# vasudeva-ram/Julia-NewtonRaphsonHANK

Hardware: AMD Instinct MI355X
Metric: sequence-space JVPs/sec (household block: BackwardIteration+ForwardIteration+aggregation, Krusell-Smith T=300) (higher is better)
Workload: dtype f64; 1 GPU; ks_2000x11_T300_N32; grid=2000x11, T=300, tangents_per_gpu=32, step=1 dual-sweep pass: primal + N tangents (hank_primal_jvp), parallelism=tangent-sharded x1

## Files before the change

include/hank_hip.h:

```cpp
#ifndef HANK_HIP_H
#define HANK_HIP_H

#include <stdint.h>

#ifdef __cplusplus
extern "C" {
#endif

typedef struct hank_ctx hank_ctx;

enum {
    HANK_OK = 0,
    HANK_ERR_NO_DEVICE = 1,
    HANK_ERR_BAD_ARG = 2,
    HANK_ERR_KNOTS = 3,
    HANK_ERR_DOMAIN = 4,
    HANK_ERR_NOT_READY = 5,
    HANK_ERR_NONMONOTONE = 6,
    HANK_ERR_NOMEM = 7,
    HANK_ERR_SWEEP = 8,
    HANK_ERR_LAUNCH = 9
};

enum {
// ... 28 lines not shown
int hank_primal(hank_ctx *ctx, const double *xhh, double *agg_out);
int hank_jvp(hank_ctx *ctx, const double *dxhh, int32_t N, double *dagg_out);

int hank_primal_dev(hank_ctx *ctx, const double *d_xhh, double *d_agg_out);
int hank_jvp_dev(hank_ctx *ctx, const double *d_dxhh, int32_t N, double *d_dagg_out);
int hank_check(hank_ctx *ctx);

int hank_primal_jvp(hank_ctx *ctx, const double *xhh, const double *dxhh, int32_t N, double *agg_out,
                    double *dagg_out);
int hank_primal_jvp_dev(hank_ctx *ctx, const double *d_xhh, const double *d_dxhh, int32_t N,
                        double *d_agg_out, double *d_dagg_out);

int hank_get_policy_seq(hank_ctx *ctx, double *out);
int hank_get_dpolicy_seq(hank_ctx *ctx, int32_t N, double *out);
int hank_get_lottery_record(hank_ctx *ctx, int32_t *lo, double *lw, double *ig, void *lq, double *iga);
int hank_get_het_outputs(hank_ctx *ctx, int32_t n_het, const double *dxhh, int32_t N, double *agg_out, double *dagg_out);
int hank_get_het_outputs_dev(hank_ctx *ctx, int32_t n_het, const double *d_dxhh, int32_t N, double *d_agg_out, double *d_dagg_out);
int hank_set_het_outputs(hank_ctx *ctx, int32_t n_het);
int hank_get_grid_aggregates(hank_ctx *ctx, double *agg2_out, int32_t N, double *dagg2_out);
int hank_get_grid_aggregates_dev(hank_ctx *ctx, double *d_agg2_out, int32_t N, double *d_dagg2_out);
int hank_get_dist_seq(hank_ctx *ctx, double *out);

int hank_backward_step(hank_ctx *ctx, const double *value_next, const double *xhh_t,
                       double *value_out, double *policy_out);
int hank_backward_step_dual(hank_ctx *ctx, const double *value_next, const double *dvalue_next,
                            const double *xhh_t, const double *dxhh_t, int32_t N,
                            double *value_out, double *dvalue_out, double *policy_out,
                            double *dpolicy_out);
int hank_forward_step(hank_ctx *ctx, const double *policy, const double *D_prev, double *D_out,
                      double *agg_out);
// ... 64 lines not shown
```

julia-newtonraphsonhank_amd/csrc/hank_device.h:

```cpp
#pragma once
#include <hip/hip_runtime.h>
#include <stdint.h>
#include "hank_geom.h"

#ifndef HANK_XFWD_LQ
#define HANK_XFWD_LQ 1
#endif
#ifndef HANK_XFWD_EARLY_BATCH
#define HANK_XFWD_EARLY_BATCH 0
#endif

namespace hank {

struct Consts {
    int n_a, n_e, G, P;
    int n_hh;
    int diet;
    double beta, gamma, bc;
    const double *a, *z, *Pi;
};

struct Record {
    double *s, *kc, *A, *B, *u, *v, *pol, *lw, *ig, *Dseq;
    int *ib, *lo, *start, *clo;
// ... 487 lines not shown
template <typename VT>
struct AdjHx<VT, 0> {};

struct SsCtl { int stop, iters; double resid; };

enum { ERR_KNOTS = 3, ERR_DOMAIN = 4, ERR_NONMONO = 6 };

__device__ inline void set_err(int *err, int code, int t, int e, int j) {
    if (atomicCAS(&err[0], 0, code) == 0) {
        err[1] = t;
        err[2] = e;
        err[3] = j;
    }
}

__device__ __forceinline__ void lottery_body(const Consts &c, const Record &R, int col, int *err, int write_seg, int use_ib, int *shlo, int *sh_clo, int4 *lq = nullptr) {
    const int t = col / c.n_e, e = col % c.n_e;
    const size_t base = (size_t)col * c.n_a;
    const int n = c.n_a;
    if (threadIdx.x == 0) *sh_clo = 0;
    __syncthreads();
    for (int j = threadIdx.x; j < n; j += blockDim.x) {
        const double p = R.pol[base + j];
        int lo = -1, hi = n;
        if (use_ib) {
            const int g0 = min(max(R.ib[base + j], 0), n - 2);
            const double a0 = c.a[g0], a1 = c.a[g0 + 1];
            if (a0 < p && p <= a1) { lo = g0; hi = g0 + 1; }
            else if (g0 > 0 && p <= a0 && c.a[g0 - 1] < p) { lo = g0 - 1; hi = g0; }
        }
// ... 2 lines not shown
            if (c.a[mid] < p) lo = mid; else hi = mid;
        }
        int l;
        double w, ig;
        if (hi == 0) {
            l = 0; w = 0.0; ig = 0.0;
            atomicMax(sh_clo, j + 1);
        } else if (hi >= n) {
            l = n - 2; w = 1.0; ig = 0.0;
        } else {
            l = hi - 1;
            const double gap = c.a[hi] - c.a[l];
            w = (p - c.a[l]) / gap;
            ig = 1.0 / gap;
        }
        R.lo[base + j] = l; R.lw[base + j] = w; R.ig[base + j] = ig;
        if (lq) lq[base + j] = make_int4(__double2loint(w), __double2hiint(w), l, (hi == 0 || hi >= n) ? 1 : 0);
        shlo[j] = (hi == 0) ? -1 : l;
    }
    __syncthreads();
    const int clo = *sh_clo;
    if (threadIdx.x == 0) R.clo[col] = clo;
    int *st = R.start + (size_t)col * (n + 1);
    int *shst = shlo + n;
    for (int j = threadIdx.x; j < n; j += blockDim.x) {
        const int prev = j ? shlo[j - 1] : -1, cur = shlo[j];
        if (cur < prev) set_err(err, ERR_NONMONO, t, e, j);
        for (int r = (prev < 0 ? 0 : prev + 1); r <= cur; r++) shst[r] = j;
        if (j == n - 1)
            for (int r = (cur < 0 ? 0 : cur + 1); r <= n; r++) shst[r] = n;
    }
    __syncthreads();
    for (int r = threadIdx.x; r <= n; r += blockDim.x) st[r] = shst[r];
    if (write_seg)
        for (int r = threadIdx.x; r < n; r += blockDim.x)
            R.seg[base + r] = make_int4(r > 0 ? shst[r - 1] : shst[r], shst[r], shst[r + 1], 0);
}

struct AdjLane { int e, nl, rl, RB, m; bool mok; };
__device__ __forceinline__ AdjLane adj_lane(const AdjGeom &g) {
    AdjLane L;
    const int lane = threadIdx.x & 63;
    L.e = __builtin_amdgcn_readfirstlane((int)(threadIdx.x >> 6));
    L.nl = lane & (g.NC - 1); L.rl = lane >> g.lgNC; L.RB = 64 >> g.lgNC;
    L.m = blockIdx.y * g.NC + L.nl;
    L.mok = L.m < g.MV;
    return L;
}

template <typename VT, typename Load, typename Begin, typename Src>
__device__ __forceinline__ void adj_dist_body(const Consts &c, const Record &R, const AdjGeom &g, const AdjLane &L, int t, double *adj_sh, Load load,
// ... 152 lines not shown
```

julia-newtonraphsonhank_amd/csrc/hank_hip.hip:

```cpp
#include "hank_kernels.h"
#include "hank_xsweep.h"
#include "hank_xspec.h"
#include "hank_jacobian.h"
#include "hank_wide.h"
#include "hank_hetx.h"
#include "hank_scen.h"
#include "hank_ssbatch.h"
#include "hank_adjoint.h"
#include "hank_boundary.h"
#include "hank_ssdiff_launch.h"
#include "../../include/hank_hip.h"

#include <cstdarg>
#include <cstdio>
#include <cstdlib>
#include <cstring>
#include <initializer_list>
#include <list>
#include <mutex>
#include <new>
#include <vector>

using namespace hank;

// ... 69 lines not shown
    DevBuf<double> dagg_pass;
    DevBuf<double> dagg_cm;
};
struct XWork {
    bool ready = false;
    int grid = 0, Sact = 0, maxt = 768, dmax = XD_MAX;
    DevBuf<XSync> sync;
    DevBuf<double> st_s, st_ds, st_D, st_dD;
    DevBuf<double> Dvirt, aggpart, rho;
    DevBuf<double> D0own;
    DevBuf<int> srcB, srcF;
    DevBuf<int2> unitsF;
    DevBuf<int> unit_overflow;
    int ucap = 64;
    bool rng_valid = false;
    bool neigh = true;
    bool syncwave = true;
    int lds_max = 65536;
    int fault_where = 7;
    int fault = 0;
    bool src_valid = false;
    std::list<XTan> tans;
    int last_blocks = 0;
    int xspec = XSPEC_CRRA;
    int inst[4] = {-1, -1, -1, -1};
};

struct WTan {
    int N = 0;
    DevBuf<double> dxhh;
// ... 94 lines not shown
    int schedule = 2;
    bool forced_xcd = false;
    TanBatch batch;
    int xjvp_max = 64;
    XWork xw;
    struct { DevBuf<double> dpT, iota, E, Cp, F, Dv, W, dsum; int N = 0, n_het = 0; } fn;
    int wide_mode = 0, wide_min = 80, num_cus = 256, wide_r = 2;
    size_t lds_max = 65536;
    DevBuf<char> rec_slab;
    size_t rec_bytes = 0;
    int4 *rec_lq = nullptr;
    double *rec_iga = nullptr;
    DevBuf<int> d_ibw;
    bool seg_valid = true;
    bool lwg_valid = true;
    long long lwg_builds = 0;
    bool wprep_valid = false;
    std::list<WTan> wtans;
    std::list<CotWork> cws;
    CotBatch cot;
    DevBuf<int> d_adj_sb;
    bool adj_seg_valid = false;
    DevBuf<double> d_bnd_q;
    HxRecord hx;
    ScenWork scen;
    int scen_pending = 0;
    std::vector<double> h_Pi, h_z;
    long long stats[N_STATS] = {};
    bool memo_on = true;
    bool xdual_back = true;
// ... 15 lines not shown
static void cot_none(hank_ctx *ctx) { ctx->cot = CotBatch(); }
static void cot_ran(hank_ctx *ctx, const void *ws, int M, const double *pbar) { ctx->cot = CotBatch{true, M, ws, pbar}; }
static void batch_ran(hank_ctx *ctx, int family, const void *ws, int N, const double *dagg_cm, const double *dpol, const std::vector<XPass> *passes = nullptr) {
    ctx->batch = TanBatch{family, true, N, ws, dagg_cm, dpol, passes};
}
static void batch_ran_boundary(hank_ctx *ctx, const void *ws, int N, const double *dagg_cm, const double *dpol, const double *zm) {
    batch_ran(ctx, 0, ws, N, dagg_cm, dpol);
    ctx->batch.boundary = true;
    ctx->batch.bnd_zm = zm;
}
static int batch_current(hank_ctx *ctx, int N, const TanBatch **out) {
    if (!ctx->batch.current || ctx->batch.N != N) return fail(ctx, HANK_ERR_NOT_READY, "no tangent sweep with N=%d is current", N);
    *out = &ctx->batch;
    return HANK_OK;
}
static void record_rewritten(hank_ctx *ctx, bool seg_written, bool lwg_written) {
    ctx->primal_done = true; ctx->seg_valid = seg_written; ctx->lwg_valid = lwg_written;
    ctx->wprep_valid = false; ctx->xw.src_valid = false; ctx->xw.rng_valid = false; ctx->adj_seg_valid = false; ctx->hx.valid = false;
    batch_none(ctx);
    cot_none(ctx);
}
static void record_gone(hank_ctx *ctx) {
    record_rewritten(ctx, false, false);
    ctx->primal_done = false;
}
static hipError_t join_side(hank_ctx *ctx) {
    if (!ctx->side_pending) return hipSuccess;
    ctx->side_pending = false;
    return hipStreamWaitEvent(ctx->stream, ctx->ev_side, 0);
}

static int fail(hank_ctx *ctx, int code, const char *fmt, ...) {
// ... 446 lines not shown
    HIPC(ctx, hipMemsetAsync(X.sync, 0, sizeof(XSync) * ((size_t)2 + 2 * XPASS_MAX), ctx->stream));
    HIPC(ctx, X.st_s.alloc(2 * XG * G));
    HIPC(ctx, X.st_ds.alloc(2 * XG * G * X.dmax));
    const size_t GM = (size_t)c.n_e * X.Sact * 64;
    HIPC(ctx, X.st_D.alloc(2 * XG * std::max(GV, GM)));
    HIPC(ctx, X.st_dD.alloc(2 * XG * GM * xslots(X.dmax + 1).SP));
    HIPC(ctx, X.Dvirt.alloc(P * c.n_e * 64));
    HIPC(ctx, X.D0own.alloc(P * c.n_e));
    HIPC(ctx, X.aggpart.alloc(2 * P * (size_t)X.Sact));
    HIPC(ctx, X.rho.alloc(P));
    HIPC(ctx, X.srcB.alloc(P * X.Sact));
    HIPC(ctx, X.srcF.alloc(P * X.Sact));
    HIPC(ctx, X.unitsF.alloc(P * X.Sact * XUCAP));
    HIPC(ctx, X.unit_overflow.alloc(1));
    HIPC(ctx, hipMemsetAsync(X.unit_overflow, 0, sizeof(int), ctx->stream));
    if (const char *ng = getenv("HANK_XNEIGH")) X.neigh = atoi(ng) != 0;
    if (const char *uc = getenv("HANK_XUCAP")) X.ucap = std::min(XUCAP, std::max(1, atoi(uc)));
    {
        double ms = 20.0;
        if (const char *wm = getenv("HANK_XWAIT_MS")) ms = atof(wm);
        const unsigned long long ticks = (unsigned long long)(std::max(ms, 0.01) * 1e5);
        HIPC(ctx, hipMemcpyToSymbol(HIP_SYMBOL(hank::g_xwait_ticks), &ticks, sizeof(ticks)));
    }
    if (const char *sv = getenv("HANK_XSYNCWAVE")) X.syncwave = atoi(sv) != 0;
    X.lds_max = (int)prop.sharedMemPerBlock;
    if (const char *xf = getenv("HANK_XFAULT")) {
        X.fault = strncmp(xf, "placement", 9) == 0 ? XERR_PLACEMENT : (strncmp(xf, "timeout", 7) == 0 ? XERR_TIMEOUT : (strncmp(xf, "stall", 5) == 0 ? 3 : 0));
        const char *w = strchr(xf, ':');
        X.fault_where = !w ? 7 : (strcmp(w, ":primal") == 0 ? 1 : (strcmp(w, ":tangent") == 0 ? 2 : (strcmp(w, ":fixedpoint") == 0 ? 4 : 7)));
    }
// ... 56 lines not shown
    }
    auto by_d = [&](auto ne, auto crra) {
        constexpr int NE = decltype(ne)::value, CRRA = decltype(crra)::value;
        if (D == 1) XL(k_xdual_back<1, 768, NE, CRRA>);
        else if (D == 2) XL(k_xdual_back<2, 768, NE, CRRA>);
        else XL(k_xdual_back<4, 768, NE, CRRA>);
    };
    auto by_crra = [&](auto ne) {
        if (sp.crra) by_d(ne, std::integral_constant<int, 1>()); else if constexpr (decltype(ne)::value != 0) by_d(ne, std::integral_constant<int, 0>());
    };
    if (sp.ne == 4) by_crra(std::integral_constant<int, 4>());
    else if (sp.ne == 7) by_crra(std::integral_constant<int, 7>());
    else if (sp.ne == 11) by_crra(std::integral_constant<int, 11>());
    else by_crra(std::integral_constant<int, 0>());
}
static void x_launch_fwd(XSection &sec, XWork &X, const Consts &c, int D, bool val, const XSweepFwdArgs &a) {
    if (val && D > 0) { X.inst[2] = 0; X.inst[3] = 0; }
#if HANK_XFWD_LQ
    if (val && D > 0 && x_lds_fwd_lq(c, D) <= (size_t)X.lds_max) {
        const size_t lds = x_lds_fwd_lq(c, D);
        x_by_maxt(X, [&](auto mt) {
            constexpr int MT = decltype(mt)::value;
            if (D == 1) XL(k_xfwd<1, true, MT, true>);
            else if (D == 2) XL(k_xfwd<2, true, MT, true>);
            else if (D == 4) { if constexpr (MT == 768) XL(k_xfwd<4, true, MT, true>); }
        });
        return;
    }
#endif
    const size_t lds = x_lds_fwd(c, D, val || D == 0);
    x_by_maxt(X, [&](auto mt) {
        constexpr int MT = decltype(mt)::value;
        if (D == 0) XL(k_xfwd<0, true, MT>);
        else if (D == 1) { if (val) XL(k_xfwd<1, true, MT>); else XL(k_xfwd<1, false, MT>); }
        else if (D == 2) { if (val) XL(k_xfwd<2, true, MT>); else XL(k_xfwd<2, false, MT>); }
        else if (D == 4) { if constexpr (MT == 768) { if (val) XL(k_xfwd<4, true, MT>); else XL(k_xfwd<4, false, MT>); } }
    });
}
static void x_launch_primal_back(XSection &sec, const XWork &X, const Consts &c, const XBackArgs &a) { const size_t lds = x_lds_primal_back(c); x_by_maxt(X, [&](auto mt) { XL(k_xprimal_back<decltype(mt)::value>); }); }
static void x_launch_tan_back(XSection &sec, const XWork &X, const Consts &c, int D, const XTanBackArgs &a) {
    const size_t lds = x_lds_tan_back(c, D);
    x_by_maxt(X, [&](auto mt) {
        constexpr int MT = decltype(mt)::value;
        if (D == 1) XL(k_xtan_back<1, MT>);
        else if (D == 2) XL(k_xtan_back<2, MT>);
        else if (D == 4) { if constexpr (MT == 768) XL(k_xtan_back<4, MT>); }
    });
}
static void x_ensure_rng(XSection &sec) {
    hank_ctx *ctx = sec.ctx;
    XWork &X = ctx->xw;
    if (X.rng_valid) return;
    hipLaunchKernelGGL(k_xunits_fwd, dim3((unsigned)ctx->c.P, (unsigned)X.Sact), dim3(256), 0, sec.stream(), ctx->c, ctx->R, X.Sact, X.srcF, X.unitsF, X.unit_overflow, X.ucap);
    X.rng_valid = true;
}

static int ensure_seg(hank_ctx *ctx) {
    if (ctx->seg_valid) return HANK_OK;
    hipLaunchKernelGGL(k_seg_build, dim3((unsigned)(ctx->c.P * ctx->c.n_e)), dim3(256), 0, ctx->stream, ctx->c, ctx->R, ctx->c.P * ctx->c.n_e);
    HIPC(ctx, hipGetLastError());
    ctx->seg_valid = true;
    return HANK_OK;
}
static int ensure_lwg(hank_ctx *ctx) {
    if (ctx->lwg_valid) return HANK_OK;
    const XWork &X = ctx->xw;
    hipLaunchKernelGGL(k_xlwg_build, dim3((unsigned)(ctx->c.P * ctx->c.n_e)), dim3(256), 0, ctx->stream, ctx->c, ctx->R, X.Dvirt, X.D0own, X.Sact);
    HIPC(ctx, hipGetLastError());
    ctx->lwg_valid = true;
    ctx->lwg_builds++;
    return HANK_OK;
}
static int x_sync_reset(XSection &sec, XSync *base, int count, int where) {
    hank_ctx *ctx = sec.ctx;
    HIPC(ctx, hipMemsetAsync(base, 0, sizeof(XSync) * (size_t)count, sec.stream()));
    if (ctx->xw.fault && ctx->xw.fault != 3 && (ctx->xw.fault_where & where)) hipLaunchKernelGGL(k_xpoison, dim3(1), dim3(64), 0, sec.stream(), base, count, (unsigned)ctx->xw.fault);
    return HANK_OK;
}

static void x_rho(XSection &sec) {
// ... 46 lines not shown
        x_launch_dual_back(sec, X, c, ps.D, db);
    } else x_launch_primal_back(sec, X, c, ab);
    HIPC(ctx, ctx->spans.end(PRIMAL_BACK, sec.stream(), 1));
    return HANK_OK;
}
static void x_lottery(XSection &sec, bool seg, bool lq = false) {
    hank_ctx *ctx = sec.ctx;
    const Consts &c = ctx->c;
#if HANK_XFWD_LQ
    if (lq) {
        hipLaunchKernelGGL(k_lottery_lq, dim3((unsigned)(c.P * c.n_e)), dim3(256), sizeof(int) * (2 * (size_t)c.n_a + 2), sec.stream(), c, ctx->R, c.P * c.n_e, ctx->d_err, seg ? 1 : 0, 1, ctx->rec_lq);
        return;
    }
#endif
    hipLaunchKernelGGL(k_lottery, dim3((unsigned)(c.P * c.n_e)), dim3(256), sizeof(int) * (2 * (size_t)c.n_a + 2), sec.stream(), c, ctx->R, c.P * c.n_e, ctx->d_err, seg ? 1 : 0, 1);
}
static int x_tan_back(XSection &sec, XTan *w) {
    hank_ctx *ctx = sec.ctx; XWork &X = ctx->xw;
    const int np = (int)w->passes.size();
    XTanBackArgs ab{};
    ab.c = ctx->c; ab.R = ctx->R; ab.rho = X.rho; ab.xhh = ctx->d_xhh; ab.dxr = w->dxr; ab.dxw = w->dxw; ab.dxt = w->dxt; ab.Ntot = w->N; ab.st_ds = X.st_ds;
    ab.src = X.neigh ? X.srcB.get() : nullptr;
    ab.stall = X.fault == 3 ? 1 : 0;
    HIPC(ctx, ctx->spans.begin(TAN_BACK, sec.stream()));
    for (int p = 0; p < np; p++) {
        const XPass &ps = w->passes[p];
        ab.n0 = ps.n0; ab.N = ps.N; ab.groups = ps.groups; ab.sy = X.sync + 2 + 2 * p; ab.dpol = w->dpol + ps.dpol_off;
        x_launch_tan_back(sec, X, ctx->c, ps.D, ab);
    }
    HIPC(ctx, ctx->spans.end(TAN_BACK, sec.stream(), np));
// ... 345 lines not shown
        ctx->forced_xcd = true;
    }
    if (const char *wr = getenv("HANK_WIDE_R")) ctx->wide_r = atoi(wr) == 4 ? 4 : 2;
    ctx->wide_mode = (w_supported(ctx) && !(se && (strcmp(se, "launch") == 0 || strcmp(se, "xcd") == 0))) ? 1 : 0;
    if (se && strcmp(se, "wide") == 0) {
        if (!w_supported(ctx))
            return fail(ctx, HANK_ERR_BAD_ARG, "HANK_SCHEDULE=wide: %dx%d, T=%d does not fit the on-chip wide sweeps (n_e instantiated: 2,3,4,5,7,11; n_a <= %d; %zu bytes of LDS per workgroup, the device has %zu)",
                        c.n_a, c.n_e, ctx->T, WIDE_CS, w_lds(ctx), ctx->lds_max);
        ctx->wide_mode = 2;
    }
    if (const char *wm = getenv("HANK_WIDE_MIN")) ctx->wide_min = std::max(1, atoi(wm));
    if (const char *xm = getenv("HANK_XJVP_MAX")) ctx->xjvp_max = atoi(xm);
    if (const char *pm = getenv("HANK_PRIMAL_MEMO")) ctx->memo_on = atoi(pm) != 0;
    if (const char *xd = getenv("HANK_XDUAL_BACK")) ctx->xdual_back = atoi(xd) != 0;
    ctx->xw.xspec = x_spec_mode(getenv("HANK_XSPEC"));
    int rc = HANK_OK;
    if (ctx->schedule == 0) rc = build_primal_graphs(ctx);
    else rc = x_setup(ctx);
    if (rc) return rc;
    ctx->errmsg[0] = 0;
    return HANK_OK;
}

int hank_destroy(hank_ctx *ctx) {
    if (!ctx) return HANK_OK;
    ENTER(ctx);
    if (ctx->side_stream) (void)hipStreamSynchronize(ctx->side_stream);
    if (ctx->own_stream) (void)hipStreamSynchronize(ctx->own_stream);
    if (ctx->ev_stream) (void)hipEventDestroy(ctx->ev_stream);
    if (ctx->ev_fork) (void)hipEventDestroy(ctx->ev_fork);
// ... 184 lines not shown
    HIPC(ctx, sec.opened());
    if (prologue) {
        hipLaunchKernelGGL(k_xdual_prologue, dim3(64), dim3(256), 0, sec.stream(), xhh, ctx->d_xhh, dxhh, w->dxhh, ctx->c.n_hh, ctx->c.P, w->N, X.rho, w->dxr, w->dxw, w->dxt,
                           reinterpret_cast<xv4u *>(X.sync.get()), sizeof(XSync) * 4 / sizeof(xv4u), ctx->d_err);
    } else {
        HIPC(ctx, hipMemcpyAsync(w->dxhh, dxhh, sizeof(double) * nP * w->N, kind, sec.stream()));
        HIPC(ctx, hipMemcpyAsync(ctx->d_xhh, xhh, sizeof(double) * nP, kind, sec.stream()));
        int rc = x_sync_reset(sec, X.sync, 2, 1);
        if (!rc) rc = x_sync_reset(sec, X.sync + 2, 2, 2);
        if (rc) return rc;
        zero_err(ctx, sec.stream());
        x_rho(sec);
        x_tan_in(sec, w);
    }
    int rc = x_back(sec, w); if (rc) return rc;
    x_lottery(sec, false, true);
    record_rewritten(ctx, false, false);
    x_ensure_rng(sec);
    HIPC(ctx, ctx->spans.begin(TAN_BACK, sec.stream()));
    HIPC(ctx, ctx->spans.end(TAN_BACK, sec.stream(), 1));
    HIPC(ctx, ctx->spans.begin(TAN_FWD, sec.stream()));
    rc = x_tan_fwd(sec, w, 0, true); if (rc) return rc;
    HIPC(ctx, ctx->spans.end(TAN_FWD, sec.stream(), 1));
    x_dual_epilogue(sec, w, d_agg_out, d_dagg_out);
    HIPC(ctx, hipGetLastError());
    HIPC(ctx, sec.close());
    x_dual_ran(ctx, w, 2);
    return HANK_OK;
}
static bool x_dual_back_fits(const hank_ctx *ctx, int D);
static int x_dual(hank_ctx *ctx, const double *xhh, const double *dxhh, hipMemcpyKind kind, int N, double *d_agg_out, double *d_dagg_out) {
    int rc = x_setup(ctx); if (rc) return rc;
    XTan *w = nullptr;
// ... 494 lines not shown
    if (!ctx || !out) return HANK_ERR_BAD_ARG;
    ENTER(ctx);
    if (!ctx->primal_done) return fail(ctx, HANK_ERR_NOT_READY, "no primal sweep has been run");
    HIPC(ctx, join_side(ctx));
    HIPC(ctx, hipMemcpyAsync(out, ctx->R.pol, sizeof(double) * (size_t)ctx->c.P * ctx->c.G, hipMemcpyDeviceToHost, ctx->stream));
    HIPC(ctx, hipStreamSynchronize(ctx->stream));
    return HANK_OK;
}

int hank_get_lottery_record(hank_ctx *ctx, int32_t *lo, double *lw, double *ig, void *lq, double *iga) {
    if (!ctx) return HANK_ERR_BAD_ARG;
    ENTER(ctx);
    if (!ctx->primal_done) return fail(ctx, HANK_ERR_NOT_READY, "no primal sweep has been run");
    if ((lq || iga) && !ctx->rec_lq) return fail(ctx, HANK_ERR_BAD_ARG, "hank_get_lottery_record: this build keeps no packed lottery record");
    HIPC(ctx, join_side(ctx));
    const size_t n = (size_t)ctx->c.P * ctx->c.G;
    if (lo) HIPC(ctx, hipMemcpyAsync(lo, ctx->R.lo, sizeof(int) * n, hipMemcpyDeviceToHost, ctx->stream));
    if (lw) HIPC(ctx, hipMemcpyAsync(lw, ctx->R.lw, sizeof(double) * n, hipMemcpyDeviceToHost, ctx->stream));
    if (ig) HIPC(ctx, hipMemcpyAsync(ig, ctx->R.ig, sizeof(double) * n, hipMemcpyDeviceToHost, ctx->stream));
    if (lq) HIPC(ctx, hipMemcpyAsync(lq, ctx->rec_lq, sizeof(int4) * n, hipMemcpyDeviceToHost, ctx->stream));
    if (iga) HIPC(ctx, hipMemcpyAsync(iga, ctx->rec_iga, sizeof(double) * (size_t)ctx->c.n_a, hipMemcpyDeviceToHost, ctx->stream));
    HIPC(ctx, hipStreamSynchronize(ctx->stream));
    return HANK_OK;
}

int hank_get_dist_seq(hank_ctx *ctx, double *out) {
    if (!ctx || !out) return HANK_ERR_BAD_ARG;
    ENTER(ctx);
    if (!ctx->primal_done) return fail(ctx, HANK_ERR_NOT_READY, "no primal sweep has been run");
    HIPC(ctx, join_side(ctx));
    HIPC(ctx, hipMemcpyAsync(out, ctx->R.Dseq + ctx->c.G, sizeof(double) * (size_t)ctx->c.P * ctx->c.G, hipMemcpyDeviceToHost, ctx->stream));
    HIPC(ctx, hipStreamSynchronize(ctx->stream));
    return HANK_OK;
}

static int grid_aggregates(hank_ctx *ctx, double *agg2_out, int32_t N, double *dagg2_out, bool dev) {
// ... 95 lines not shown
    HIPC(ctx, hipStreamBeginCapture(s, hipStreamCaptureModeThreadLocal));
    int cur = 0;
    for (int t = 0; t < P; t++) {
        hipLaunchKernelGGL((k_adj_egm<VT>), grd, blk, ldsB, s, c, ctx->R, w.g, t, t == 0 ? 1 : 0, t == P - 1 ? 1 : 0, ctx->d_adj_sb, st[cur], st[cur ^ 1], pbar,
                           reinterpret_cast<VT *>(w.partS.get()), reinterpret_cast<VT *>(w.partM.get()));
        cur ^= 1;
    }
    hipLaunchKernelGGL(k_adj_out, dim3((unsigned)((P * w.N + 255) / 256)), dim3(256), 0, s, P, c.n_hh, w.N, w.g.nb, ctx->d_xhh, w.partS, w.partM, w.yb1,
                       ctx->d_agg + P, ctx->d_zd, w.xbar);
    return end_capture(ctx, &w.g_B);
}

static int ensure_adj_seg(hank_ctx *ctx) {
    const Consts &c = ctx->c;
    if (ctx->adj_seg_valid) return HANK_OK;
    hipLaunchKernelGGL(k_adj_seg, dim3((unsigned)(c.P * c.n_e)), dim3(256), sizeof(int) * ((size_t)c.n_a + 1), ctx->stream, c, ctx->R, c.P * c.n_e, ctx->d_adj_sb);
    HIPC(ctx, hipGetLastError());
    ctx->adj_seg_valid = true;
    return HANK_OK;
}

static int ensure_hx_record(hank_ctx *ctx) {
    const Consts &c = ctx->c;
    HxRecord &h = ctx->hx;
    if (h.valid) return HANK_OK;
    const size_t P = c.P, SX = hx_count(ctx);
    if (!h.S) {
        HIPC(ctx, h.f.alloc(SX * P * c.G));
        HIPC(ctx, h.fc.alloc(SX * P * c.G));
        HIPC(ctx, h.S.alloc(P * SX * HX_NS));
    }
    hipLaunchKernelGGL(k_hx_record, dim3((unsigned)P, (unsigned)SX), dim3(256), 0, ctx->stream, c, ctx->R, ctx->d_xhh, (int)SX, h.f.get(), h.fc.get(), h.S.get());
    HIPC(ctx, hipGetLastError());
    h.valid = true;
    return HANK_OK;
}

static int enqueue_vjp(hank_ctx *ctx, int n_het, const double *agg_bar, hipMemcpyKind kind, int M, double *d_xhh_bar, CotWork **out,
                       double *d_vend_bar = nullptr, double *d_D0_bar = nullptr) {
    const Consts &c = ctx->c;
// ... 1062 lines not shown
```

julia-newtonraphsonhank_amd/csrc/hank_xsweep.h:

```cpp
#pragma once
#include "hank_kernels.h"
#include "hank_xaddr.h"
#include "hank_xlds.h"
#include <type_traits>

namespace hank {

constexpr int XG = 8;
constexpr int XRW = 63;
enum { XERR_TIMEOUT = 1, XERR_PLACEMENT = 2 };
__device__ unsigned long long g_xwait_ticks = 2000000ull;
struct XDeadline {
    unsigned long long t0;
    __device__ __forceinline__ XDeadline() : t0(__builtin_amdgcn_s_memrealtime()) {}
    __device__ __forceinline__ bool expired(unsigned spins) const { return (spins & 63u) == 63u && __builtin_amdgcn_s_memrealtime() - t0 > g_xwait_ticks; }
    __device__ __forceinline__ unsigned waited_us() const { return (unsigned)((__builtin_amdgcn_s_memrealtime() - t0) / 100ull); }
};

struct XSync {
    unsigned ticket[XG][32];
    unsigned total[32];
    unsigned flag[XG][64][32];
    unsigned status[32];
    unsigned pad[32];
// ... 1519 lines not shown
        units[((size_t)t * Sact + m) * XUCAP + k] = su[e][k - soff[e]];
    }
    if (threadIdx.x == 0) {
        int tot = soff[ne], anyclo = 0, anyopen = 0;
        for (int e = 0; e < ne; e++) {
            if (sclo[e] > 0) anyclo = 1; else anyopen = 1;
        }
        if (tot > ucap) { atomicExch(overflow, 1); tot = min(tot, XUCAP); }
        int ml = min(slo, m), mh = max(shi, m);
        if (sany0) { ml = 0; mh = Sact - 1; }
        const int allv = (m == 0 && vnz && anyopen) ? 1 : 0;
        src[(size_t)t * Sact + m] = ml | (mh << 8) | (anyclo << 16) | (allv << 17) | (tot << 18);
    }
}

__global__ void k_xsrc_back(Consts c, Record R, int Sact, int *src) {
    __shared__ int smin[256], smax[256];
    const int t = blockIdx.x, m = blockIdx.y;
    const int r0 = m * XRW, rows = min(XRW, c.n_a - r0);
    int lo = 1 << 30, hi = -1;
    for (int k = threadIdx.x; k < rows * c.n_e; k += blockDim.x) {
        const int e = k / rows, a = r0 + (k - e * rows);
        const size_t ro = (size_t)t * c.G + (size_t)e * c.n_a + a;
        if (R.A[ro] != 0.0 || R.B[ro] != 0.0) { const int ib = R.ib[ro]; lo = min(lo, ib); hi = max(hi, ib + 1); }
    }
    smin[threadIdx.x] = lo; smax[threadIdx.x] = hi;
    __syncthreads();
    if (threadIdx.x == 0) {
        for (int k = 1; k < (int)blockDim.x; k++) { lo = min(lo, smin[k]); hi = max(hi, smax[k]); }
        int ml = m, mh = m;
// ... 126 lines not shown
```

julia-newtonraphsonhank_amd/hip.py:

```python
from __future__ import annotations

import ctypes as C
from pathlib import Path

import numpy as np

import os

_LIB_PATH = Path(os.environ.get("HANK_HIP_LIB") or Path(__file__).resolve().parent / "libhank_hip.so")
_lib = None

HANK_OK = 0
HANK_ERR_NO_DEVICE, HANK_ERR_BAD_ARG, HANK_ERR_KNOTS, HANK_ERR_DOMAIN = 1, 2, 3, 4
HANK_ERR_NOT_READY, HANK_ERR_NONMONOTONE, HANK_ERR_NOMEM, HANK_ERR_SWEEP, HANK_ERR_LAUNCH = 5, 6, 7, 8, 9
HANK_VF_KRUSELL_SMITH = 0

ABI_SYMBOLS = (
    "hank_create", "hank_create_on", "hank_gather_columns", "hank_destroy", "hank_last_error", "hank_n_hh", "hank_set_stream", "hank_sync",
    "hank_set_boundary", "hank_primal", "hank_jvp", "hank_primal_dev", "hank_jvp_dev", "hank_check",
    "hank_primal_jvp", "hank_primal_jvp_dev",
    "hank_get_policy_seq", "hank_get_dpolicy_seq", "hank_get_dist_seq", "hank_get_het_outputs", "hank_get_het_outputs_dev", "hank_set_het_outputs",
    "hank_get_grid_aggregates", "hank_get_grid_aggregates_dev", "hank_backward_step",
    "hank_backward_step_dual", "hank_forward_step", "hank_forward_step_dual", "hank_last_timings", "hank_stats", "hank_info", "hank_sweep_instance", "hank_vfi", "hank_stationary_dist", "hank_fake_news", "hank_fake_news_het", "hank_device_available",
    "hank_vjp", "hank_vjp_dev", "hank_get_policy_cotangent_seq", "hank_last_vjp_timings", "hank_vjp_het", "hank_vjp_het_dev",
    "hank_jvp_boundary", "hank_jvp_boundary_dev", "hank_vjp_boundary", "hank_vjp_boundary_dev",
    "hank_jvp_het", "hank_jvp_het_dev", "hank_vjp_het_boundary", "hank_vjp_het_boundary_dev",
    "hank_ss_jvp", "hank_ss_jvp_dev", "hank_ss_vjp", "hank_ss_vjp_dev", "hank_last_ss_timings",
    "hank_primal_batch", "hank_primal_batch_dev", "hank_last_batch_timings",
    "hank_ss_batch", "hank_last_ss_batch_timings",
    "hank_get_lottery_record",
)


class HankHIPError(RuntimeError):

    def __init__(self, code: int, msg: str):
        super().__init__(f"[hank_hip status {code}] {msg}")
        self.code = code


class KnotsNotSortedError(HankHIPError):
    """Interpolations.jl's 'knot-vectors must be unique and sorted' (KrusellSmith.jl:69-72)."""


class DomainError(HankHIPError):
# ... 43 lines not shown
    lib.hank_set_stream.argtypes = [vp, vp]
    lib.hank_sync.argtypes = [vp]
    lib.hank_set_boundary.argtypes = [vp, dp, dp]
    lib.hank_primal.argtypes = [vp, dp, dp]
    lib.hank_jvp.argtypes = [vp, dp, i32, dp]
    lib.hank_primal_dev.argtypes = [vp, vp, vp]
    lib.hank_jvp_dev.argtypes = [vp, vp, i32, vp]
    lib.hank_check.argtypes = [vp]
    lib.hank_primal_jvp.argtypes = [vp, dp, dp, i32, dp, dp]
    lib.hank_primal_jvp_dev.argtypes = [vp, vp, vp, i32, vp, vp]
    lib.hank_get_policy_seq.argtypes = [vp, dp]
    lib.hank_get_dpolicy_seq.argtypes = [vp, i32, dp]
    lib.hank_get_dist_seq.argtypes = [vp, dp]
    if hasattr(lib, "hank_get_lottery_record"):
        lib.hank_get_lottery_record.argtypes = [vp, vp, dp, dp, vp, dp]
    lib.hank_get_het_outputs.argtypes = [vp, i32, dp, i32, dp, dp]
    lib.hank_get_het_outputs_dev.argtypes = [vp, i32, vp, i32, vp, vp]
    lib.hank_set_het_outputs.argtypes = [vp, i32]
    lib.hank_get_grid_aggregates.argtypes = [vp, dp, i32, dp]
    lib.hank_get_grid_aggregates_dev.argtypes = [vp, vp, i32, vp]
    lib.hank_backward_step.argtypes = [vp, dp, dp, dp, dp]
    lib.hank_backward_step_dual.argtypes = [vp, dp, dp, dp, dp, i32, dp, dp, dp, dp]
    lib.hank_forward_step.argtypes = [vp, dp, dp, dp, dp]
    lib.hank_forward_step_dual.argtypes = [vp, dp, dp, dp, dp, i32, dp, dp, dp, dp]
    lib.hank_last_timings.argtypes = [vp, dp, C.POINTER(i32)]
    lib.hank_stats.argtypes = [vp, C.POINTER(C.c_int64)]
    lib.hank_info.argtypes = [vp, C.POINTER(C.c_int64)]
    lib.hank_sweep_instance.argtypes = [vp, C.POINTER(i32)]
    lib.hank_vfi.argtypes = [vp, dp, C.c_double, i32, dp, dp, C.POINTER(i32), dp]
    lib.hank_stationary_dist.argtypes = [vp, dp, dp, C.c_double, i32, i32, C.POINTER(i32)]
# ... 13 lines not shown
    lib.hank_jvp_het.argtypes = [vp, i32, dp, dp, dp, i32, dp]
    lib.hank_jvp_het_dev.argtypes = [vp, i32, vp, vp, vp, i32, vp]
    lib.hank_vjp_het_boundary.argtypes = [vp, i32, dp, i32, dp, dp, dp]
    lib.hank_vjp_het_boundary_dev.argtypes = [vp, i32, vp, i32, vp, vp, vp]
    lib.hank_ss_jvp.argtypes = [vp, i32, dp, i32, C.c_double, i32, dp, dp, dp, dp, C.POINTER(i32), dp]
    lib.hank_ss_jvp_dev.argtypes = [vp, i32, vp, i32, C.c_double, i32, vp, vp, vp, vp, C.POINTER(i32), dp]
    lib.hank_ss_vjp.argtypes = [vp, i32, dp, dp, dp, i32, C.c_double, i32, dp, C.POINTER(i32), dp]
    lib.hank_ss_vjp_dev.argtypes = [vp, i32, vp, vp, vp, i32, C.c_double, i32, vp, C.POINTER(i32), dp]
    lib.hank_last_ss_timings.argtypes = [vp, dp]
    lib.hank_primal_batch.argtypes = [vp, i32, dp, i32, dp, dp, C.POINTER(i32)]
    lib.hank_primal_batch_dev.argtypes = [vp, i32, vp, i32, vp, vp]
    lib.hank_last_batch_timings.argtypes = [vp, dp]
    lib.hank_ss_batch.argtypes = [vp, i32, dp, i32, C.c_double, i32, C.c_double, i32, i32, dp, dp, dp, dp, C.POINTER(i32), dp, C.POINTER(i32)]
    lib.hank_last_ss_batch_timings.argtypes = [vp, dp]
    for name in ABI_SYMBOLS:
        if name == "hank_get_lottery_record" and not hasattr(lib, name):
            continue
        if name != "hank_last_error":
            getattr(lib, name).restype = C.c_int
    _lib = lib
    return lib


def device_available() -> bool:
    try:
        return bool(load_library().hank_device_available())
    except (RuntimeError, OSError):
        return False


def gather_columns(blocks, d_block_ptrs, N_k, d_out_ptr: int):
# ... 402 lines not shown
        return {"back": (int(out[0]), int(out[1])), "fwd": (int(out[2]), int(out[3]))}

    def policy_seq(self) -> np.ndarray:
        out = np.empty((self.n_a, self.n_e, self.P), order="F")
        self._chk(self._lib.hank_get_policy_seq(self._ctx, _p(out)))
        return out

    def lottery_record(self):
        shp = (self.n_a, self.n_e, self.P)
        lo, lw, ig = np.empty(shp, np.int32, order="F"), np.empty(shp, order="F"), np.empty(shp, order="F")
        lq = np.empty(shp, np.dtype([("w", "<f8"), ("lo", "<i4"), ("flags", "<i4")]), order="F")
        iga = np.empty(self.n_a)
        self._chk(self._lib.hank_get_lottery_record(self._ctx, lo.ctypes.data_as(C.c_void_p), _p(lw), _p(ig), lq.ctypes.data_as(C.c_void_p), _p(iga)))
        return {"lo": lo, "lw": lw, "ig": ig, "lq": lq, "iga": iga}

    def dist_seq(self) -> np.ndarray:
        out = np.empty((self.n_a, self.n_e, self.P), order="F")
        self._chk(self._lib.hank_get_dist_seq(self._ctx, _p(out)))
        return out

    def dpolicy_seq(self, N: int) -> np.ndarray:
        out = np.empty((self.n_a, self.n_e, self.P, N), order="F")
        self._chk(self._lib.hank_get_dpolicy_seq(self._ctx, int(N), _p(out)))
        return out

    def het_outputs(self, n_het: int = 2, dxhh=None):
        agg = np.empty((self.P, n_het), order="F")
        if dxhh is None:
            self._chk(self._lib.hank_get_het_outputs(self._ctx, int(n_het), None, 0, _p(agg), None))
            return agg, None
# ... 97 lines not shown
```

Baseline: 9205 JVPs/s.

## Fuse lottery build with forward work-unit cutting in a lean front kernel

Between the backward and forward dual sweeps, the separate lottery kernel and forward-units kernel are replaced by a fused front kernel. It computes the lottery in a lean mode that skips writing the lo/lw/ig/start/seg arrays and cuts per-column work units into staging buffers, followed by a small pack kernel that builds the unit lists. The full lottery record is now rebuilt lazily by ensure_lottery only when other paths need it. This is meant to cut global memory writes and a launch on the JVP critical path. In exchange it adds staging buffers, new invalidation state and a lazy-rebuild cost on other APIs.

```diff
diff --git a/include/hank_hip.h b/include/hank_hip.h
--- a/include/hank_hip.h
+++ b/include/hank_hip.h
@@ -66,6 +66,7 @@
 int hank_get_policy_seq(hank_ctx *ctx, double *out);
 int hank_get_dpolicy_seq(hank_ctx *ctx, int32_t N, double *out);
 int hank_get_lottery_record(hank_ctx *ctx, int32_t *lo, double *lw, double *ig, void *lq, double *iga);
+int hank_get_forward_units(hank_ctx *ctx, int32_t *src, int32_t *units);
 int hank_get_het_outputs(hank_ctx *ctx, int32_t n_het, const double *dxhh, int32_t N, double *agg_out, double *dagg_out);
 int hank_get_het_outputs_dev(hank_ctx *ctx, int32_t n_het, const double *d_dxhh, int32_t N, double *d_agg_out, double *d_dagg_out);
 int hank_set_het_outputs(hank_ctx *ctx, int32_t n_het);
diff --git a/julia-newtonraphsonhank_amd/csrc/hank_device.h b/julia-newtonraphsonhank_amd/csrc/hank_device.h
--- a/julia-newtonraphsonhank_amd/csrc/hank_device.h
+++ b/julia-newtonraphsonhank_amd/csrc/hank_device.h
@@ -525,6 +525,7 @@
     }
 }
 
+template <bool LEAN = false>
 __device__ __forceinline__ void lottery_body(const Consts &c, const Record &R, int col, int *err, int write_seg, int use_ib, int *shlo, int *sh_clo, int4 *lq = nullptr) {
     const int t = col / c.n_e, e = col % c.n_e;
     const size_t base = (size_t)col * c.n_a;
@@ -557,7 +558,7 @@
             w = (p - c.a[l]) / gap;
             ig = 1.0 / gap;
         }
-        R.lo[base + j] = l; R.lw[base + j] = w; R.ig[base + j] = ig;
+        if constexpr (!LEAN) { R.lo[base + j] = l; R.lw[base + j] = w; R.ig[base + j] = ig; }
         if (lq) lq[base + j] = make_int4(__double2loint(w), __double2hiint(w), l, (hi == 0 || hi >= n) ? 1 : 0);
         shlo[j] = (hi == 0) ? -1 : l;
     }
@@ -574,10 +575,27 @@
             for (int r = (cur < 0 ? 0 : cur + 1); r <= n; r++) shst[r] = n;
     }
     __syncthreads();
+    if constexpr (LEAN) return;
     for (int r = threadIdx.x; r <= n; r += blockDim.x) st[r] = shst[r];
     if (write_seg)
         for (int r = threadIdx.x; r < n; r += blockDim.x)
             R.seg[base + r] = make_int4(r > 0 ? shst[r - 1] : shst[r], shst[r], shst[r + 1], 0);
+}
+
+__device__ __forceinline__ int lottery_hi(const Consts &c, const Record &R, size_t idx, double p, int use_ib) {
+    const int n = c.n_a;
+    int lo = -1, hi = n;
+    if (use_ib) {
+        const int g0 = min(max(R.ib[idx], 0), n - 2);
+        const double a0 = c.a[g0], a1 = c.a[g0 + 1];
+        if (a0 < p && p <= a1) { lo = g0; hi = g0 + 1; }
+        else if (g0 > 0 && p <= a0 && c.a[g0 - 1] < p) { lo = g0 - 1; hi = g0; }
+    }
+    while (hi - lo > 1) {
+        const int mid = lo + ((hi - lo) >> 1);
+        if (c.a[mid] < p) lo = mid; else hi = mid;
+    }
+    return hi;
 }
 
 struct AdjLane { int e, nl, rl, RB, m; bool mok; };
diff --git a/julia-newtonraphsonhank_amd/csrc/hank_hip.hip b/julia-newtonraphsonhank_amd/csrc/hank_hip.hip
--- a/julia-newtonraphsonhank_amd/csrc/hank_hip.hip
+++ b/julia-newtonraphsonhank_amd/csrc/hank_hip.hip
@@ -107,6 +107,10 @@
     DevBuf<int> unit_overflow;
     int ucap = 64;
     bool rng_valid = false;
+    DevBuf<int2> stageU;
+    DevBuf<int4> stageM;
+    bool front = true;
+    int front_poison = 0;
     bool neigh = true;
     bool syncwave = true;
     int lds_max = 65536;
@@ -231,6 +235,7 @@
     DevBuf<int> d_ibw;
     bool seg_valid = true;
     bool lwg_valid = true;
+    bool lot_valid = true;
     long long lwg_builds = 0;
     bool wprep_valid = false;
     std::list<WTan> wtans;
@@ -276,8 +281,8 @@
     *out = &ctx->batch;
     return HANK_OK;
 }
-static void record_rewritten(hank_ctx *ctx, bool seg_written, bool lwg_written) {
-    ctx->primal_done = true; ctx->seg_valid = seg_written; ctx->lwg_valid = lwg_written;
+static void record_rewritten(hank_ctx *ctx, bool seg_written, bool lwg_written, bool lot_written = true) {
+    ctx->primal_done = true; ctx->seg_valid = seg_written && lot_written; ctx->lwg_valid = lwg_written && lot_written; ctx->lot_valid = lot_written;
     ctx->wprep_valid = false; ctx->xw.src_valid = false; ctx->xw.rng_valid = false; ctx->adj_seg_valid = false; ctx->hx.valid = false;
     batch_none(ctx);
     cot_none(ctx);
@@ -754,6 +759,10 @@
     HIPC(ctx, X.unitsF.alloc(P * X.Sact * XUCAP));
     HIPC(ctx, X.unit_overflow.alloc(1));
     HIPC(ctx, hipMemsetAsync(X.unit_overflow, 0, sizeof(int), ctx->stream));
+    if (X.front && ctx->rec_lq) {
+        HIPC(ctx, X.stageU.alloc(P * X.Sact * c.n_e * XU_ROWS));
+        HIPC(ctx, X.stageM.alloc(P * X.Sact * c.n_e));
+    }
     if (const char *ng = getenv("HANK_XNEIGH")) X.neigh = atoi(ng) != 0;
     if (const char *uc = getenv("HANK_XUCAP")) X.ucap = std::min(XUCAP, std::max(1, atoi(uc)));
     {
@@ -840,10 +849,17 @@
     else if (sp.ne == 11) by_crra(std::integral_constant<int, 11>());
     else by_crra(std::integral_constant<int, 0>());
 }
+static bool x_fwd_serves_lq(const XWork &X, const Consts &c, int D) {
+#if HANK_XFWD_LQ
+    return D > 0 && x_lds_fwd_lq(c, D) <= (size_t)X.lds_max;
+#else
+    return false;
+#endif
+}
 static void x_launch_fwd(XSection &sec, XWork &X, const Consts &c, int D, bool val, const XSweepFwdArgs &a) {
     if (val && D > 0) { X.inst[2] = 0; X.inst[3] = 0; }
 #if HANK_XFWD_LQ
-    if (val && D > 0 && x_lds_fwd_lq(c, D) <= (size_t)X.lds_max) {
+    if (val && x_fwd_serves_lq(X, c, D)) {
         const size_t lds = x_lds_fwd_lq(c, D);
         x_by_maxt(X, [&](auto mt) {
             constexpr int MT = decltype(mt)::value;
@@ -873,16 +889,26 @@
         else if (D == 4) { if constexpr (MT == 768) XL(k_xtan_back<4, MT>); }
     });
 }
+static int ensure_lottery(hank_ctx *ctx, hipStream_t s = nullptr) {
+    if (ctx->lot_valid) return HANK_OK;
+    const Consts &c = ctx->c;
+    hipLaunchKernelGGL(k_lottery, dim3((unsigned)(c.P * c.n_e)), dim3(256), sizeof(int) * (2 * (size_t)c.n_a + 2), s ? s : ctx->stream, c, ctx->R, c.P * c.n_e, ctx->d_err, 0, 1);
+    HIPC(ctx, hipGetLastError());
+    ctx->lot_valid = true;
+    return HANK_OK;
+}
 static void x_ensure_rng(XSection &sec) {
     hank_ctx *ctx = sec.ctx;
     XWork &X = ctx->xw;
     if (X.rng_valid) return;
+    (void)ensure_lottery(ctx, sec.stream());
     hipLaunchKernelGGL(k_xunits_fwd, dim3((unsigned)ctx->c.P, (unsigned)X.Sact), dim3(256), 0, sec.stream(), ctx->c, ctx->R, X.Sact, X.srcF, X.unitsF, X.unit_overflow, X.ucap);
     X.rng_valid = true;
 }
 
 static int ensure_seg(hank_ctx *ctx) {
     if (ctx->seg_valid) return HANK_OK;
+    { const int rc = ensure_lottery(ctx); if (rc) return rc; }
     hipLaunchKernelGGL(k_seg_build, dim3((unsigned)(ctx->c.P * ctx->c.n_e)), dim3(256), 0, ctx->stream, ctx->c, ctx->R, ctx->c.P * ctx->c.n_e);
     HIPC(ctx, hipGetLastError());
     ctx->seg_valid = true;
@@ -890,6 +916,7 @@
 }
 static int ensure_lwg(hank_ctx *ctx) {
     if (ctx->lwg_valid) return HANK_OK;
+    { const int rc = ensure_lottery(ctx); if (rc) return rc; }
     const XWork &X = ctx->xw;
     hipLaunchKernelGGL(k_xlwg_build, dim3((unsigned)(ctx->c.P * ctx->c.n_e)), dim3(256), 0, ctx->stream, ctx->c, ctx->R, X.Dvirt, X.D0own, X.Sact);
     HIPC(ctx, hipGetLastError());
@@ -966,6 +993,14 @@
     }
 #endif
     hipLaunchKernelGGL(k_lottery, dim3((unsigned)(c.P * c.n_e)), dim3(256), sizeof(int) * (2 * (size_t)c.n_a + 2), sec.stream(), c, ctx->R, c.P * c.n_e, ctx->d_err, seg ? 1 : 0, 1);
+}
+static void x_front(XSection &sec) {
+    hank_ctx *ctx = sec.ctx; XWork &X = ctx->xw;
+    const Consts &c = ctx->c;
+    hipLaunchKernelGGL(k_xdual_front, dim3((unsigned)(c.P * c.n_e)), dim3(512), sizeof(int) * (2 * (size_t)c.n_a + 2), sec.stream(), c, ctx->R, c.P * c.n_e, ctx->d_err, ctx->rec_lq,
+                       X.Sact, X.stageU.get(), X.stageM.get(), X.front_poison);
+    hipLaunchKernelGGL(k_xunits_pack, dim3((unsigned)((c.P * X.Sact + 3) / 4)), dim3(256), 0, sec.stream(), c, ctx->R, X.Sact, X.stageU.get(), X.stageM.get(), X.srcF.get(), X.unitsF.get(),
+                       X.unit_overflow.get(), X.ucap);
 }
 static int x_tan_back(XSection &sec, XTan *w) {
     hank_ctx *ctx = sec.ctx; XWork &X = ctx->xw;
@@ -1341,6 +1376,8 @@
     if (const char *pm = getenv("HANK_PRIMAL_MEMO")) ctx->memo_on = atoi(pm) != 0;
     if (const char *xd = getenv("HANK_XDUAL_BACK")) ctx->xdual_back = atoi(xd) != 0;
     ctx->xw.xspec = x_spec_mode(getenv("HANK_XSPEC"));
+    if (const char *xf = getenv("HANK_XDUAL_FRONT")) ctx->xw.front = atoi(xf) != 0;
+    if (const char *xp = getenv("HANK_XDUAL_FRONT_POISON")) ctx->xw.front_poison = atoi(xp) != 0 ? 1 : 0;
     int rc = HANK_OK;
     if (ctx->schedule == 0) rc = build_primal_graphs(ctx);
     else rc = x_setup(ctx);
@@ -1555,9 +1592,15 @@
         x_tan_in(sec, w);
     }
     int rc = x_back(sec, w); if (rc) return rc;
-    x_lottery(sec, false, true);
-    record_rewritten(ctx, false, false);
-    x_ensure_rng(sec);
+    if (X.front && X.stageU && ctx->rec_lq && x_fwd_serves_lq(X, ctx->c, w->passes[0].D)) {
+        x_front(sec);
+        record_rewritten(ctx, false, false, false);
+        X.rng_valid = true;
+    } else {
+        x_lottery(sec, false, true);
+        record_rewritten(ctx, false, false);
+        x_ensure_rng(sec);
+    }
     HIPC(ctx, ctx->spans.begin(TAN_BACK, sec.stream()));
     HIPC(ctx, ctx->spans.end(TAN_BACK, sec.stream(), 1));
     HIPC(ctx, ctx->spans.begin(TAN_FWD, sec.stream()));
@@ -2082,12 +2125,26 @@
     if (!ctx->primal_done) return fail(ctx, HANK_ERR_NOT_READY, "no primal sweep has been run");
     if ((lq || iga) && !ctx->rec_lq) return fail(ctx, HANK_ERR_BAD_ARG, "hank_get_lottery_record: this build keeps no packed lottery record");
     HIPC(ctx, join_side(ctx));
+    if (lo || lw || ig) { const int rc = ensure_lottery(ctx); if (rc) return rc; }
     const size_t n = (size_t)ctx->c.P * ctx->c.G;
     if (lo) HIPC(ctx, hipMemcpyAsync(lo, ctx->R.lo, sizeof(int) * n, hipMemcpyDeviceToHost, ctx->stream));
     if (lw) HIPC(ctx, hipMemcpyAsync(lw, ctx->R.lw, sizeof(double) * n, hipMemcpyDeviceToHost, ctx->stream));
     if (ig) HIPC(ctx, hipMemcpyAsync(ig, ctx->R.ig, sizeof(double) * n, hipMemcpyDeviceToHost, ctx->stream));
     if (lq) HIPC(ctx, hipMemcpyAsync(lq, ctx->rec_lq, sizeof(int4) * n, hipMemcpyDeviceToHost, ctx->stream));
     if (iga) HIPC(ctx, hipMemcpyAsync(iga, ctx->rec_iga, sizeof(double) * (size_t)ctx->c.n_a, hipMemcpyDeviceToHost, ctx->stream));
+    HIPC(ctx, hipStreamSynchronize(ctx->stream));
+    return HANK_OK;
+}
+
+int hank_get_forward_units(hank_ctx *ctx, int32_t *src, int32_t *units) {
+    if (!ctx) return HANK_ERR_BAD_ARG;
+    ENTER(ctx);
+    const XWork &X = ctx->xw;
+    if (!ctx->primal_done || !X.ready || !X.rng_valid) return fail(ctx, HANK_ERR_NOT_READY, "hank_get_forward_units: no persistent sweep has cut the recorded lottery into work units");
+    HIPC(ctx, join_side(ctx));
+    const size_t n = (size_t)ctx->c.P * X.Sact;
+    if (src) HIPC(ctx, hipMemcpyAsync(src, X.srcF, sizeof(int) * n, hipMemcpyDeviceToHost, ctx->stream));
+    if (units) HIPC(ctx, hipMemcpyAsync(units, X.unitsF, sizeof(int2) * n * XUCAP, hipMemcpyDeviceToHost, ctx->stream));
     HIPC(ctx, hipStreamSynchronize(ctx->stream));
     return HANK_OK;
 }
@@ -2213,6 +2270,7 @@
 static int ensure_adj_seg(hank_ctx *ctx) {
     const Consts &c = ctx->c;
     if (ctx->adj_seg_valid) return HANK_OK;
+    { const int rc = ensure_lottery(ctx); if (rc) return rc; }
     hipLaunchKernelGGL(k_adj_seg, dim3((unsigned)(c.P * c.n_e)), dim3(256), sizeof(int) * ((size_t)c.n_a + 1), ctx->stream, c, ctx->R, c.P * c.n_e, ctx->d_adj_sb);
     HIPC(ctx, hipGetLastError());
     ctx->adj_seg_valid = true;
@@ -2223,6 +2281,7 @@
     const Consts &c = ctx->c;
     HxRecord &h = ctx->hx;
     if (h.valid) return HANK_OK;
+    { const int rc = ensure_lottery(ctx); if (rc) return rc; }
     const size_t P = c.P, SX = hx_count(ctx);
     if (!h.S) {
         HIPC(ctx, h.f.alloc(SX * P * c.G));
diff --git a/julia-newtonraphsonhank_amd/csrc/hank_xsweep.h b/julia-newtonraphsonhank_amd/csrc/hank_xsweep.h
--- a/julia-newtonraphsonhank_amd/csrc/hank_xsweep.h
+++ b/julia-newtonraphsonhank_amd/csrc/hank_xsweep.h
@@ -2,6 +2,7 @@
 #include "hank_kernels.h"
 #include "hank_xaddr.h"
 #include "hank_xlds.h"
+#include "hank_xunits.h"
 #include <type_traits>
 
 namespace hank {
@@ -1557,6 +1558,78 @@
     }
 }
 
+static_assert(XU_ROWS == XRW && XU_LANES == 64, "hank_xunits.h cuts for this sweep geometry");
+__global__ void __launch_bounds__(512) k_xdual_front(Consts c, Record R, int ncols, int *err, int4 *lq, int Sact, int2 *su, int4 *sm, int poison) {
+    extern __shared__ int shlo[];
+    __shared__ int sh_clo, sh_vnz;
+    const int col = blockIdx.x;
+    if (col >= ncols) return;
+    const int ne = c.n_e, n = c.n_a;
+    const int t = col / ne, e = col - t * ne;
+    bool v = false;
+    if (t > 0 && (int)threadIdx.x < ne) {
+        const size_t i0 = (size_t)(t - 1) * c.G + (size_t)threadIdx.x * n;
+        v = lottery_hi(c, R, i0, R.pol[i0], 1) == 0;
+    }
+    if (threadIdx.x == 0) sh_vnz = 0;
+    lottery_body<true>(c, R, col, err, 0, 1, shlo, &sh_clo, lq);
+    if (v) atomicOr(&sh_vnz, 1);
+    if (poison) {
+        const size_t base = (size_t)col * n;
+        const double qnan = __longlong_as_double(0x7ff8000000000000ll);
+        for (int j = threadIdx.x; j < n; j += blockDim.x) { R.lo[base + j] = 0; R.lw[base + j] = qnan; R.ig[base + j] = qnan; }
+        for (int r = threadIdx.x; r <= n; r += blockDim.x) R.start[(size_t)col * (n + 1) + r] = 0;
+    }
+    __syncthreads();
+    const int *shst = shlo + n;
+    const int clo = sh_clo;
+    const bool vnz = sh_vnz != 0;
+    const int lane = threadIdx.x & 63, wave = threadIdx.x >> 6, nwaves = blockDim.x >> 6;
+    auto S = [&](int r) { return min(max(shst[min(max(r, 0), n)], 0), n); };
+    for (int m = wave + nwaves * lane; m < Sact; m += nwaves * 64) {
+        const int r0 = m * XRW, nrows = min(XRW, n - r0);
+        const size_t slot = ((size_t)t * Sact + m) * ne + e;
+        int2 *out = su + slot * XU_ROWS;
+        const XuCut q = xu_cut(S, [&](int ta) { return xu_next(S, clo, vnz, Sact, r0, nrows, ta); }, [&](int k, int x, int y) { out[k] = make_int2(x, y); },
+                               clo, vnz, r0, nrows, Sact, e, m, XU_ROWS);
+        sm[slot] = make_int4(q.n, q.mlo, q.mhi, q.anyv);
+    }
+}
+__global__ void __launch_bounds__(256) k_xunits_pack(Consts c, Record R, int Sact, const int2 *su, const int4 *sm, int *src, int2 *units, int *overflow, int ucap) {
+    const int lane = threadIdx.x & 63, w = blockIdx.x * (blockDim.x >> 6) + (threadIdx.x >> 6);
+    if (w >= c.P * Sact) return;
+    const int ne = c.n_e, t = w / Sact, m = w - t * Sact;
+    int4 q = make_int4(0, m, m, 0);
+    int clo = 0, clop = 0;
+    if (lane < ne) {
+        q = sm[(size_t)w * ne + lane];
+        clo = R.clo[(size_t)t * ne + lane];
+        clop = t > 0 ? R.clo[(size_t)(t - 1) * ne + lane] : 0;
+    }
+    const int cnt = min(max(q.x, 0), XU_ROWS);
+    int inc = cnt;
+    for (int off = 1; off < 64; off <<= 1) { const int up = __shfl_up(inc, off, 64); if (lane >= off) inc += up; }
+    const int excl = inc - cnt;
+    int tot = __shfl(inc, 63, 64);
+    int mycol = -1, myoff = 0;
+    for (int e = 0; e < ne; e++) {
+        const int oe = __shfl(excl, e, 64), ce = __shfl(cnt, e, 64);
+        if (lane >= oe && lane < oe + ce) { mycol = e; myoff = lane - oe; }
+    }
+    if (mycol >= 0 && lane < XUCAP) units[(size_t)w * XUCAP + lane] = su[((size_t)w * ne + mycol) * XU_ROWS + myoff];
+    int ml = min(q.y, m), mh = max(q.z, m);
+    for (int off = 32; off > 0; off >>= 1) { ml = min(ml, __shfl_xor(ml, off, 64)); mh = max(mh, __shfl_xor(mh, off, 64)); }
+    const bool sany0 = __ballot(lane < ne && q.w != 0) != 0, anyclo = __ballot(lane < ne && clo > 0) != 0;
+    const bool anyopen = __ballot(lane < ne && clo <= 0) != 0, vnz = __ballot(clop > 0) != 0;
+    if (lane == 0) {
+        if (tot > ucap) { atomicExch(overflow, 1); tot = min(tot, XUCAP); }
+        ml = min(max(ml, 0), Sact - 1); mh = min(max(mh, 0), Sact - 1);
+        if (sany0) { ml = 0; mh = Sact - 1; }
+        const int allv = (m == 0 && vnz && anyopen) ? 1 : 0;
+        src[w] = ml | (mh << 8) | ((anyclo ? 1 : 0) << 16) | (allv << 17) | (tot << 18);
+    }
+}
+
 __global__ void k_xsrc_back(Consts c, Record R, int Sact, int *src) {
     __shared__ int smin[256], smax[256];
     const int t = blockIdx.x, m = blockIdx.y;
diff --git a/julia-newtonraphsonhank_amd/csrc/hank_xunits.h b/julia-newtonraphsonhank_amd/csrc/hank_xunits.h
--- /dev/null
+++ b/julia-newtonraphsonhank_amd/csrc/hank_xunits.h
@@ -0,0 +1,81 @@
+#pragma once
+
+#if defined(__HIPCC__)
+#define XU_FN __host__ __device__ __forceinline__
+#else
+#define XU_FN static inline
+#endif
+
+namespace hank {
+
+constexpr int XU_ROWS = 63;
+constexpr int XU_LANES = 64;
+
+XU_FN int xu_min(int a, int b) { return a < b ? a : b; }
+XU_FN int xu_max(int a, int b) { return a > b ? a : b; }
+
+struct XuCut { int n, mlo, mhi, anyv; };
+
+XU_FN void xu_encode(int e, int ja, int cnt, int ta, int tb, int nv, int *x, int *y) {
+    *x = e | (ja << 4) | (cnt << 16);
+    *y = ta | (tb << 8) | (nv << 16);
+}
+
+template <typename S>
+XU_FN int xu_lanes(S s, int clo, bool vnz, int r0, int a, int b, int *ja_out, bool *has0_out) {
+    const int ja = s(r0 + a - 1 < 0 ? 0 : r0 + a - 1);
+    *ja_out = ja;
+    *has0_out = ja == 0 && clo <= 0 && vnz;
+    return xu_max(s(r0 + b) - ja, 0);
+}
+template <typename S>
+XU_FN bool xu_fits(S s, int ja, bool has0, int Sact, int r0, int b) {
+    const int c2 = xu_max(s(r0 + b) - ja, 0);
+    return c2 + ((has0 && c2 > 0) ? Sact : 0) <= XU_LANES;
+}
+template <typename S>
+XU_FN int xu_next(S s, int clo, bool vnz, int Sact, int r0, int nrows, int a) {
+    int ja; bool has0;
+    (void)xu_lanes(s, clo, vnz, r0, a, a + 1, &ja, &has0);
+    auto fits = [&](int b) { return xu_fits(s, ja, has0, Sact, r0, b); };
+    int lo = a + 1, hi = nrows;
+    if (lo < hi && fits(lo + 1)) {
+        if (fits(hi)) lo = hi;
+        else {
+            lo = lo + 1;
+            while (hi - lo > 1) { const int mid = (lo + hi) >> 1; if (fits(mid)) lo = mid; else hi = mid; }
+        }
+    }
+    return lo;
+}
+template <typename S, typename Next, typename Emit>
+XU_FN XuCut xu_cut(S s, Next next, Emit emit, int clo, bool vnz, int r0, int nrows, int Sact, int e, int m, int cap) {
+    XuCut q;
+    q.n = 0; q.mlo = m; q.mhi = m; q.anyv = 0;
+    int ta = 0;
+    while (ta < nrows && q.n < cap) {
+        const int tb = xu_min(xu_max(next(ta), ta + 1), nrows);
+        int ja; bool has0;
+        const int cnt = xu_lanes(s, clo, vnz, r0, ta, tb, &ja, &has0);
+        const int nv = (has0 && cnt > 0) ? Sact : 0;
+        if (cnt > 0) {
+            int x, y;
+            xu_encode(e, ja, cnt, ta, tb, nv, &x, &y);
+            emit(q.n, x, y);
+            q.mlo = xu_min(q.mlo, ja / XU_ROWS); q.mhi = xu_max(q.mhi, (ja + cnt - 1) / XU_ROWS);
+            if (nv) q.anyv = 1;
+            q.n++;
+        }
+        ta = tb;
+    }
+    return q;
+}
+
+static inline XuCut xu_cut_column(const int *start, int n_a, int clo, bool vnz, int r0, int nrows, int Sact, int e, int m, int *units, int cap) {
+    auto s = [&](int r) { return xu_min(xu_max(start[xu_min(xu_max(r, 0), n_a)], 0), n_a); };
+    auto next = [&](int ta) { return xu_next(s, clo, vnz, Sact, r0, nrows, ta); };
+    auto emit = [&](int k, int x, int y) { units[2 * k] = x; units[2 * k + 1] = y; };
+    return xu_cut(s, next, emit, clo, vnz, r0, nrows, Sact, e, m, cap);
+}
+
+}
diff --git a/julia-newtonraphsonhank_amd/hip.py b/julia-newtonraphsonhank_amd/hip.py
--- a/julia-newtonraphsonhank_amd/hip.py
+++ b/julia-newtonraphsonhank_amd/hip.py
@@ -28,7 +28,7 @@
     "hank_ss_jvp", "hank_ss_jvp_dev", "hank_ss_vjp", "hank_ss_vjp_dev", "hank_last_ss_timings",
     "hank_primal_batch", "hank_primal_batch_dev", "hank_last_batch_timings",
     "hank_ss_batch", "hank_last_ss_batch_timings",
-    "hank_get_lottery_record",
+    "hank_get_lottery_record", "hank_get_forward_units",
 )
 
 
@@ -102,6 +102,8 @@
     lib.hank_get_dist_seq.argtypes = [vp, dp]
     if hasattr(lib, "hank_get_lottery_record"):
         lib.hank_get_lottery_record.argtypes = [vp, vp, dp, dp, vp, dp]
+    if hasattr(lib, "hank_get_forward_units"):
+        lib.hank_get_forward_units.argtypes = [vp, vp, vp]
     lib.hank_get_het_outputs.argtypes = [vp, i32, dp, i32, dp, dp]
     lib.hank_get_het_outputs_dev.argtypes = [vp, i32, vp, i32, vp, vp]
     lib.hank_set_het_outputs.argtypes = [vp, i32]
@@ -145,7 +147,7 @@
     lib.hank_ss_batch.argtypes = [vp, i32, dp, i32, C.c_double, i32, C.c_double, i32, i32, dp, dp, dp, dp, C.POINTER(i32), dp, C.POINTER(i32)]
     lib.hank_last_ss_batch_timings.argtypes = [vp, dp]
     for name in ABI_SYMBOLS:
-        if name == "hank_get_lottery_record" and not hasattr(lib, name):
+        if name in ("hank_get_lottery_record", "hank_get_forward_units") and not hasattr(lib, name):
             continue
         if name != "hank_last_error":
             getattr(lib, name).restype = C.c_int
@@ -578,6 +580,12 @@
         self._chk(self._lib.hank_get_lottery_record(self._ctx, lo.ctypes.data_as(C.c_void_p), _p(lw), _p(ig), lq.ctypes.data_as(C.c_void_p), _p(iga)))
         return {"lo": lo, "lw": lw, "ig": ig, "lq": lq, "iga": iga}
 
+    def forward_units(self):
+        S = (self.n_a + 62) // 63
+        src, units = np.empty((self.P, S), np.int32), np.empty((self.P, S, 64, 2), np.int32)
+        self._chk(self._lib.hank_get_forward_units(self._ctx, src.ctypes.data_as(C.c_void_p), units.ctypes.data_as(C.c_void_p)))
+        return src, units
+
     def dist_seq(self) -> np.ndarray:
         out = np.empty((self.n_a, self.n_e, self.P), order="F")
         self._chk(self._lib.hank_get_dist_seq(self._ctx, _p(out)))
```

After: 9341 JVPs/s (median of 6 runs). 1.5% higher.
